# wlsdzyzl/OnePiece

Hardware: AMD Instinct MI355X
Metric: RGB-D frames/sec fused (640x480, 5 mm voxel TSDF) (higher is better)
Workload: dtype f32

## Files before the change

__graft_entry__.py:

```python
import os
import subprocess
import sys

ROOT = os.path.dirname(os.path.abspath(__file__))
if ROOT not in sys.path:
    sys.path.insert(0, ROOT)


def build():
    subprocess.check_call(["make", "-C", os.path.join(ROOT, "onepiece_amd", "csrc"), "-B", "-j8"])
    subprocess.check_call(["make", "-C", os.path.join(ROOT, "onepiece_amd", "csrc"), "-B", "-j8", "b64"])
    subprocess.check_call(["make", "-C", os.path.join(ROOT, "oracle"), "-B"])
    subprocess.check_call(["make", "-C", os.path.join(ROOT, "host", "one_piece"), "-B"])
    subprocess.check_call(["make", "-C", os.path.join(ROOT, "examples", "cpp"), "-B"])
    lib = os.path.join(ROOT, "onepiece_amd")
    subprocess.check_call(["/opt/rocm/bin/hipcc", "--offload-arch=gfx950", "-O2", "-I", os.path.join(ROOT, "include"), os.path.join(ROOT, "tools", "prof_driver.cpp"), "-L", lib,
                           "-lonepiece_hip", "-Wl,-rpath," + lib, "-o", os.path.join(ROOT, "tools", "prof_driver.bin")])
    hostlib = os.path.join(ROOT, "host", "one_piece")
    subprocess.check_call(["/opt/rocm/bin/hipcc", "--offload-arch=gfx950", "-O2", "-I", os.path.join(ROOT, "include"), os.path.join(ROOT, "tools", "ops_driver.cpp"), "-L", lib,
                           "-lonepiece_hip", "-L", hostlib, "-lone_piece_hip_host", "-Wl,-rpath," + lib, "-Wl,-rpath," + hostlib, "-o", os.path.join(ROOT, "tools", "ops_driver.bin")])
    for tool in ("hbm_calib", "valu_ubench"):
        subprocess.check_call(["/opt/rocm/bin/hipcc", "--offload-arch=gfx950", "-O2", "-Wno-unused-result", "-Wno-unused-value", os.path.join(ROOT, "tools", tool + ".hip"), "-o", os.path.join(ROOT, "tools", tool + ".bin")])
    try:
        subprocess.check_call(["make", "-C", os.path.join(ROOT, "tests", "cpp"), "-B"])
    except (OSError, subprocess.CalledProcessError) as e:
        print("build(): test artefacts under tests/cpp not built: %s" % e, file=sys.stderr)
    subprocess.check_call([os.path.join(ROOT, "oracle", "tools", "build_ref_examples.sh")])
    import onepiece_amd
    from onepiece_amd import _lib, integration, registration, odometry, dense_slam, distributed, sequence, synthetic, tool, nearest
    lib = _lib.load()
    assert lib.op_abi_version() == 1


def smoke():
    import numpy as np
    from onepiece_amd import integration as I, registration as R, synthetic as S
    from oracle import oracle as O

    s = 4
    camt = (S.FX / s, S.FY / s, S.CX / s, S.CY / s, S.W // s, S.H // s, 1000.0)
    hcam = I.PinholeCamera()
    hcam.fx, hcam.fy, hcam.cx, hcam.cy, hcam.width, hcam.height, hcam.depth_scale = camt
    hv = I.CubeHandler(hcam, device=0, max_blocks=1 << 15)
    hv.SetVoxelResolution(0.02)
# ... 46 lines not shown
```

include/onepiece_hip.h:

```cpp
#ifndef ONEPIECE_HIP_H
#define ONEPIECE_HIP_H
#include <stddef.h>
#include <stdint.h>

#ifdef __cplusplus
extern "C" {
#endif

#define OP_ABI_VERSION 1

typedef enum {
    OP_OK = 0,
    OP_ERR_INVALID = 1,
    OP_ERR_NO_DEVICE = 2,
    OP_ERR_CAPACITY = 3,
    OP_ERR_MISMATCH = 4,
    OP_ERR_NO_NORMALS = 5,
    OP_ERR_HIP = 6
} op_status;

enum { OP_DEPTH_F32 = 0, OP_DEPTH_U16 = 1 };
enum { OP_MEM_HOST = 0, OP_MEM_DEVICE = 1 };
enum { OP_ICP_POINT_TO_POINT = 0, OP_ICP_POINT_TO_PLANE = 1 };
enum { OP_TRACK_HYBRID = 0, OP_TRACK_PHOTO = 1, OP_TRACK_DEPTH = 2 };
// ... 33 lines not shown
#define OP_MERGE_OWNER_EXCHANGE 0
#define OP_MERGE_DENSE_REDUCE 1
int op_runtime_set_option(int option, long long value);
int op_runtime_get_option(int option, long long *value);
int op_runtime_set_rccl_library(const char *path);
int op_device_alloc(size_t bytes, int device, void **device_ptr);
int op_device_write(void *device_ptr, size_t n_parts, const void *const *parts, const size_t *bytes, const size_t *offsets, int device);
int op_device_upload(const void *host, size_t bytes, int device, void **device_ptr);
int op_device_release(void *device_ptr, int device);
int op_release_cached_memory(void);
int op_device_count(int *count);
int op_camera_preset(int type, op_camera *out);

int op_mat4_inverse(const float m[16], float out[16]);
uint64_t op_hash_key(int32_t x, int32_t y, int32_t z);
int op_frustum_planes(const op_camera *cam, const float pose[16], float far_dist, float near_dist,
                      float planes[24]);
int op_frustum_from_camera(const op_camera *cam, const float pose[16], float far_dist, float near_dist,
                           float planes[24], float corners[24]);
int op_frustum_from_vectors(const float forward[3], const float position[3], const float right[3],
                            const float up[3], float far_dist, float near_dist, float fov, float aspect,
                            float planes[24], float corners[24]);
int op_get_sdf(const op_camera *cam, const float point[3], const float pose[16], const float *pose_inv,
               const void *depth, int depth_fmt, float *sdf);
int op_debug_project_px(float a, float c, int fast);
int op_debug_project_uv(float fx, float fy, float cx, float cy, const float *X, const float *Y, const float *Z,
                        size_t n, int device, int32_t *out);
int op_debug_project_uv_image(float fx, float fy, float cx, float cy, int width, int height, const float *X, const float *Y,
                              const float *Z, size_t n, int device, int32_t *out);
int op_debug_voxel_update(const float *s, const float *w, const float *c0, const float *c1, const float *c2,
                          const float *new_sdf, const unsigned *rgba, long long n, float *out_fast, float *out_ref);
int op_debug_rcp(const float *x, long long n, float *out);
double op_debug_px_rcp_err(void);
int op_debug_gather2d(const unsigned *images, int width, int height, int n_frames, int frame, int column_test, const int *uv,
                      long long n, unsigned *out);
int op_se3_exp(const float x[6], float T[16]);

int op_volume_create(const op_camera *cam, float voxel_res, float truncation, float far_dist,
                     float near_dist, int device, uint64_t max_blocks, op_volume **out);
int op_volume_destroy(op_volume *v);
int op_volume_set_resolution(op_volume *v, float voxel_res);
int op_volume_set_truncation(op_volume *v, float truncation);
int op_volume_set_camera(op_volume *v, const op_camera *cam);
int op_volume_set_near_far(op_volume *v, float near_dist, float far_dist);
#define OP_VOLUME_OPT_UPDATE 0
#define OP_VOLUME_UPDATE_EXACT 0
#define OP_VOLUME_UPDATE_SUM_FORM 1
#define OP_VOLUME_OPT_SELECT 1
#define OP_VOLUME_SELECT_AUTO 0
#define OP_VOLUME_SELECT_DIRECT -1
#define OP_VOLUME_OPT_RAYCAST_PRUNE 2
int op_volume_set_option(op_volume *v, int option, int value);
int op_volume_progress(op_volume *v, uint64_t *frames_accepted, uint64_t *frames_done);
int op_volume_clear(op_volume *v);
int op_volume_sync(op_volume *v);
int op_volume_flush(op_volume *v);
int op_volume_block_count(op_volume *v, size_t *n);
int op_volume_has_cube(op_volume *v, int32_t x, int32_t y, int32_t z, int *present);
int op_volume_stream(op_volume *v, void **stream);

int op_volume_compute_bounding(op_volume *v, const void *depth, int depth_fmt, int mem,
                               const float pose[16], float max_pos[3], float min_pos[3],
                               size_t *n_inside);
int op_volume_prepare_cubes(op_volume *v, const void *depth, int depth_fmt, int mem,
                            const float pose[16], const float *pose_inv, int32_t *ids_xyz,
                            size_t cap, size_t *n, size_t *n_candidates);
// ... 248 lines not shown
```

onepiece_amd/_lib.py:

```python
import ctypes as C
import os
import subprocess

_HERE = os.path.dirname(os.path.abspath(__file__))
SO_PATH = os.environ.get("ONEPIECE_HIP_LIBRARY") or os.path.join(_HERE, "libonepiece_hip.so")
CSRC = os.path.join(_HERE, "csrc")


class OnePieceHipError(RuntimeError):
    def __init__(self, code, msg):
        super().__init__("onepiece_hip error %d: %s" % (code, msg))
        self.code = code


class Camera(C.Structure):
    _fields_ = [("fx", C.c_float), ("fy", C.c_float), ("cx", C.c_float), ("cy", C.c_float),
                ("width", C.c_int32), ("height", C.c_int32), ("depth_scale", C.c_float)]


class MergeStats(C.Structure):
    _fields_ = [("ranks", C.c_int32), ("rank", C.c_int32), ("union_blocks", C.c_uint64), ("reduce_bytes", C.c_uint64), ("slices", C.c_uint64),
                ("prepare_ms", C.c_double), ("transfer_ms", C.c_double), ("total_ms", C.c_double),
                ("algorithm", C.c_int32), ("pad_", C.c_int32), ("held_blocks", C.c_uint64), ("owned_blocks", C.c_uint64),
                ("wire_bytes_sent", C.c_uint64), ("wire_bytes_received", C.c_uint64)]
# ... 53 lines not shown
_ip = C.POINTER(C.c_int32)
_vp = C.c_void_p
_szp = C.POINTER(C.c_size_t)
_u64p = C.POINTER(C.c_uint64)

SIGNATURES = {
    "op_abi_version": (C.c_int, []),
    "op_last_error": (C.c_char_p, []),
    "op_runtime_hw_queues": (C.c_int, [C.POINTER(C.c_int)]),
    "op_runtime_configure": (C.c_int, [C.c_int]),
    "op_runtime_set_option": (C.c_int, [C.c_int, C.c_longlong]),
    "op_runtime_get_option": (C.c_int, [C.c_int, C.POINTER(C.c_longlong)]),
    "op_runtime_set_rccl_library": (C.c_int, [C.c_char_p]),
    "op_device_alloc": (C.c_int, [C.c_size_t, C.c_int, C.POINTER(_vp)]),
    "op_device_write": (C.c_int, [_vp, C.c_size_t, C.POINTER(_vp), C.POINTER(C.c_size_t), C.POINTER(C.c_size_t), C.c_int]),
    "op_device_upload": (C.c_int, [_vp, C.c_size_t, C.c_int, C.POINTER(_vp)]),
    "op_device_release": (C.c_int, [_vp, C.c_int]),
    "op_release_cached_memory": (C.c_int, []),
    "op_device_count": (C.c_int, [C.POINTER(C.c_int)]),
    "op_camera_preset": (C.c_int, [C.c_int, C.POINTER(Camera)]),
    "op_mat4_inverse": (C.c_int, [_fp, _fp]),
    "op_hash_key": (C.c_uint64, [C.c_int32, C.c_int32, C.c_int32]),
    "op_frustum_planes": (C.c_int, [C.POINTER(Camera), _fp, C.c_float, C.c_float, _fp]),
    "op_frustum_from_camera": (C.c_int, [C.POINTER(Camera), _fp, C.c_float, C.c_float, _fp, _fp]),
    "op_frustum_from_vectors": (C.c_int, [_fp, _fp, _fp, _fp, C.c_float, C.c_float, C.c_float, C.c_float, _fp, _fp]),
    "op_get_sdf": (C.c_int, [C.POINTER(Camera), _fp, _fp, _fp, _vp, C.c_int, _fp]),
    "op_se3_exp": (C.c_int, [_fp, _fp]),
    "op_debug_project_px": (C.c_int, [C.c_float, C.c_float, C.c_int]),
    "op_debug_project_uv": (C.c_int, [C.c_float, C.c_float, C.c_float, C.c_float, _vp, _vp, _vp, C.c_size_t, C.c_int, _vp]),
    "op_debug_project_uv_image": (C.c_int, [C.c_float, C.c_float, C.c_float, C.c_float, C.c_int, C.c_int, _vp, _vp, _vp, C.c_size_t, C.c_int, _vp]),
    "op_debug_voxel_update": (C.c_int, [_vp, _vp, _vp, _vp, _vp, _vp, _vp, C.c_longlong, _vp, _vp]),
    "op_debug_rcp": (C.c_int, [_vp, C.c_longlong, _vp]),
    "op_debug_px_rcp_err": (C.c_double, []),
    "op_debug_gather2d": (C.c_int, [_vp, C.c_int, C.c_int, C.c_int, C.c_int, C.c_int, _vp, C.c_longlong, _vp]),
    "op_volume_create": (C.c_int, [C.POINTER(Camera), C.c_float, C.c_float, C.c_float, C.c_float,
                                   C.c_int, C.c_uint64, C.POINTER(_vp)]),
    "op_volume_destroy": (C.c_int, [_vp]),
    "op_volume_set_resolution": (C.c_int, [_vp, C.c_float]),
    "op_volume_set_truncation": (C.c_int, [_vp, C.c_float]),
    "op_volume_set_camera": (C.c_int, [_vp, C.POINTER(Camera)]),
    "op_volume_set_near_far": (C.c_int, [_vp, C.c_float, C.c_float]),
    "op_volume_set_option": (C.c_int, [_vp, C.c_int, C.c_int]),
    "op_volume_progress": (C.c_int, [_vp, _u64p, _u64p]),
    "op_volume_clear": (C.c_int, [_vp]),
    "op_volume_sync": (C.c_int, [_vp]),
    "op_volume_flush": (C.c_int, [_vp]),
    "op_volume_block_count": (C.c_int, [_vp, _szp]),
    "op_volume_has_cube": (C.c_int, [_vp, C.c_int32, C.c_int32, C.c_int32, C.POINTER(C.c_int)]),
    "op_volume_stream": (C.c_int, [_vp, C.POINTER(_vp)]),
    "op_volume_compute_bounding": (C.c_int, [_vp, _vp, C.c_int, C.c_int, _fp, _fp, _fp, _szp]),
    "op_volume_prepare_cubes": (C.c_int, [_vp, _vp, C.c_int, C.c_int, _fp, _fp, _ip, C.c_size_t,
                                          _szp, _szp]),
    "op_volume_integrate": (C.c_int, [_vp, _vp, C.c_int, _vp, C.c_int, _fp, _fp]),
    "op_volume_integrate_sequence": (C.c_int, [_vp, _vp, C.c_size_t, C.c_int, _vp, C.c_size_t, _fp,
                                               C.c_size_t]),
    "op_volume_deintegrate": (C.c_int, [_vp, _vp, C.c_int, _vp, C.c_int, _fp, _fp]),
    "op_volume_deintegrate_sequence": (C.c_int, [_vp, _vp, C.c_size_t, C.c_int, _vp, C.c_size_t, _fp, C.c_size_t]),
    "op_volume_reintegrate": (C.c_int, [_vp, _vp, C.c_int, _vp, C.c_int, _fp, _fp]),
    "op_volume_reintegrate_sequence": (C.c_int, [_vp, _vp, C.c_size_t, C.c_int, _vp, C.c_size_t, _fp, _fp, C.c_size_t]),
    "op_volume_deintegrate_stats": (C.c_int, [_vp, _u64p, _u64p, _u64p, _u64p]),
    "op_volume_collect_garbage": (C.c_int, [_vp, C.c_float, _ip, _ip, C.POINTER(CollectStats)]),
    "op_volume_collect_last_stats": (C.c_int, [_vp, C.POINTER(CollectStats)]),
    "op_volume_integrate_cubes": (C.c_int, [_vp, _vp, C.c_int, _vp, C.c_int, _fp, _fp, _vp, C.c_size_t]),
    "op_volume_stats": (C.c_int, [_vp, _u64p, _u64p, _u64p, _u64p]),
    "op_volume_stats_launches": (C.c_int, [_vp, _u64p, _u64p, _u64p, _u64p]),
    "op_volume_growth_stats": (C.c_int, [_vp, _u64p, _u64p, _u64p]),
# ... 138 lines not shown
```

onepiece_amd/csrc/select.hip:

```cpp
#include "volume_core.hpp"

namespace {

__global__ void k_finish_select(VolView V, State* st) {
    for (unsigned k = blockIdx.x * blockDim.x + threadIdx.x; k < (unsigned)(kMaxBatch * kAccSlots * 8); k += gridDim.x * blockDim.x) (&st->acc[0][0][0])[k] = 0u;
    const unsigned n = st->n_blist < V.max_blocks ? st->n_blist : V.max_blocks;
    const unsigned nr = st->n_rec < V.max_blocks ? st->n_rec : V.max_blocks;
    for (unsigned i = blockIdx.x * blockDim.x + threadIdx.x; i < n; i += gridDim.x * blockDim.x) V.bmask[V.blist[i]] = (bmask_t)0;
    for (unsigned i = blockIdx.x * blockDim.x + threadIdx.x; i < nr; i += gridDim.x * blockDim.x) V.sel_list[i] = V.tvals[V.sel_list[i]];
}

__global__ void k_mark_cubes(VolView V, State* st, const int* __restrict__ keys, unsigned n) {
    const unsigned i = blockIdx.x * blockDim.x + threadIdx.x;
    if (i >= n || (st->overflow & 3u)) return;
    const int x = keys[3 * i], y = keys[3 * i + 1], z = keys[3 * i + 2];
    if (!key_in_range(x, y, z)) { atomicOr(&st->overflow, 8u); return; }
    bool created;
    const int slot = table_claim(V, st, x, y, z, &created);
    if (slot < 0) return;
    if (atomicOr(&V.bmask[slot], (bmask_t)1) == (bmask_t)0) {
        const unsigned pos = atomicAdd(&st->n_blist, 1u);
        if (pos < V.max_blocks) V.blist[pos] = slot;
    }
}



__global__ __launch_bounds__(256) void k_prepare_frames(KaFwd B, int f0, CamParams C, BatchPtrs Q, uint2* __restrict__ pimg, float2* __restrict__ ptile,
                                                        float* __restrict__ partial, State* st, unsigned seq,
                                                        const unsigned* __restrict__ n_blocks, unsigned* __restrict__ hstat) {
    __shared__ float s_red[4][6];
    __shared__ unsigned s_cnt[4];
    __shared__ float s_tile[4][4][2];
    const int tid = threadIdx.x, f = f0 + (int)blockIdx.y;
    if (blockIdx.x == 0 && f == 0 && tid == 0) {
        st->n_rec = 0;
        st->n_blist = 0;
        st->cur_seq = seq;
        if (hstat && (st->overflow & 3u) == 0u) {
            hstat[1] = *n_blocks;
            __threadfence_system();
            __hip_atomic_store(&hstat[0], seq - 1u, __ATOMIC_RELEASE, __HIP_MEMORY_SCOPE_SYSTEM);
        }
    }
    if (blockIdx.x == 0 && f == 0 && tid < kKcShares) st->kc_next[tid * 16] = 0u;
    if (blockIdx.x == 0 && f == 0) {
        static_assert(kKcTSlots == 256, "one slot per thread");
        unsigned long long kc = st->kc_t[tid];
        st->kc_t[tid] = 0ull;
        for (int o = 32; o > 0; o >>= 1) { const unsigned long long x = __shfl_xor(kc, o, 64); kc = x > kc ? x : kc; }
        __shared__ unsigned long long s_kc[4];
        if ((tid & 63) == 0) s_kc[tid >> 6] = kc;
        __syncthreads();
        if (tid == 0) {
            for (int w = 1; w < 4; ++w) kc = s_kc[w] > kc ? s_kc[w] : kc;
            st->stat_kc_ticks += kc;
        }
    }
    const PoseFwd& P = B.f[blockIdx.y];
    const int npix = C.width * C.height;
    const void* dptr = Q.depth[f];
    const unsigned char* cptr = Q.rgb[f];
    uint2* out = pimg + (size_t)f * npix;
    const int wgx = (C.width + kKaW - 1) / kKaW;
    const int gy = (int)blockIdx.x / wgx, gx = (int)blockIdx.x - gy * wgx;
    const int row = gy * kKaH + (tid >> 4), col0 = gx * kKaW + (tid & 15) * 4;
    float mx0 = -FLT_MAX, mx1 = -FLT_MAX, mx2 = -FLT_MAX, mn0 = FLT_MAX, mn1 = FLT_MAX, mn2 = FLT_MAX;
    float tmin = __builtin_inff(), tmax = -__builtin_inff();
    unsigned inside = 0;
    if (row < C.height && col0 < C.width) {
        const int pix0 = row * C.width + col0;
        float zz[4];
        unsigned cc[4] = {0u, 0u, 0u, 0u};
        const int nv = C.width - col0 < 4 ? C.width - col0 : 4;
        const bool wide = nv == 4 && (C.width & 3) == 0 && ((size_t)dptr & 15u) == 0 && ((size_t)cptr & 3u) == 0;
        if (wide) {
            if (C.depth_u16) {
                const ushort4 d = *reinterpret_cast<const ushort4*>((const unsigned short*)dptr + pix0);
                zz[0] = (float)d.x / C.depth_scale; zz[1] = (float)d.y / C.depth_scale; zz[2] = (float)d.z / C.depth_scale; zz[3] = (float)d.w / C.depth_scale;
            } else {
                const float4 d = *reinterpret_cast<const float4*>((const float*)dptr + pix0);
                zz[0] = d.x; zz[1] = d.y; zz[2] = d.z; zz[3] = d.w;
            }
            if (cptr) {
                const unsigned* c3 = reinterpret_cast<const unsigned*>(cptr + 3 * (size_t)pix0);
                const unsigned d0 = c3[0], d1 = c3[1], d2 = c3[2];
                cc[0] = d0 & 0xffffffu; cc[1] = (d0 >> 24) | ((d1 & 0xffffu) << 8); cc[2] = (d1 >> 16) | ((d2 & 0xffu) << 16); cc[3] = d2 >> 8;
            }
            uint4* o4 = reinterpret_cast<uint4*>(out + pix0);
            o4[0] = make_uint4(__float_as_uint(zz[0]), cc[0] | 0x01000000u, __float_as_uint(zz[1]), cc[1] | 0x01000000u);
            o4[1] = make_uint4(__float_as_uint(zz[2]), cc[2] | 0x01000000u, __float_as_uint(zz[3]), cc[3] | 0x01000000u);
        } else {
            for (int e = 0; e < nv; ++e) {
                const int pix = pix0 + e;
                zz[e] = C.depth_u16 ? (float)((const unsigned short*)dptr)[pix] / C.depth_scale : ((const float*)dptr)[pix];
                if (cptr) cc[e] = (unsigned)cptr[3 * (size_t)pix] | ((unsigned)cptr[3 * (size_t)pix + 1] << 8) | ((unsigned)cptr[3 * (size_t)pix + 2] << 16);
                out[pix] = make_uint2(__float_as_uint(zz[e]), cc[e] | 0x01000000u);
            }
        }
#pragma unroll
        for (int e = 0; e < 4; ++e) {
            if (e >= nv) break;
            const float z = zz[e];
            if (!(z > 0)) continue;
            tmin = fminf(tmin, z); tmax = fmaxf(tmax, z);
            const int i = row, j = col0 + e;
            const float x = ((float)j - C.cx) * z / C.fx;
            const float y = ((float)i - C.cy) * z / C.fy;
            const float* M = P.pose;
            const float q0 = ((M[0] * x + M[1] * y) + M[2] * z) + M[3] * 1.0f;
            const float q1 = ((M[4] * x + M[5] * y) + M[6] * z) + M[7] * 1.0f;
            const float q2 = ((M[8] * x + M[9] * y) + M[10] * z) + M[11] * 1.0f;
            const float q3 = ((M[12] * x + M[13] * y) + M[14] * z) + M[15] * 1.0f;
            float p0 = q0, p1 = q1, p2 = q2;
            if (__builtin_amdgcn_ballot_w64(q3 != 1.0f) != 0ull) { p0 = q0 / q3; p1 = q1 / q3; p2 = q2 / q3; }
            bool in = true;
#pragma unroll
            for (int k = 0; k < 6; ++k) {
                const float dist = sum3(P.planes[4 * k] * p0, P.planes[4 * k + 1] * p1, P.planes[4 * k + 2] * p2) + P.planes[4 * k + 3];
                if (dist < 0) { in = false; break; }
                if (dist == 0) break;
            }
            if (in) {
                ++inside;
                mx0 = p0 > mx0 ? p0 : mx0; mx1 = p1 > mx1 ? p1 : mx1; mx2 = p2 > mx2 ? p2 : mx2;
                mn0 = p0 < mn0 ? p0 : mn0; mn1 = p1 < mn1 ? p1 : mn1; mn2 = p2 < mn2 ? p2 : mn2;
            }
        }
    }
    tmin = fminf(tmin, __shfl_xor(tmin, 1, 64)); tmax = fmaxf(tmax, __shfl_xor(tmax, 1, 64));
    tmin = fminf(tmin, __shfl_xor(tmin, 2, 64)); tmax = fmaxf(tmax, __shfl_xor(tmax, 2, 64));
    tmin = fminf(tmin, __shfl_xor(tmin, 16, 64)); tmax = fmaxf(tmax, __shfl_xor(tmax, 16, 64));
    tmin = fminf(tmin, __shfl_xor(tmin, 32, 64)); tmax = fmaxf(tmax, __shfl_xor(tmax, 32, 64));
    mx0 = wave_max(mx0); mx1 = wave_max(mx1); mx2 = wave_max(mx2);
    mn0 = wave_min(mn0); mn1 = wave_min(mn1); mn2 = wave_min(mn2);
    inside = wave_sum(inside);
    const int wave = tid >> 6, lane = tid & 63;
    if (lane == 0) {
        s_red[wave][0] = mx0; s_red[wave][1] = mx1; s_red[wave][2] = mx2;
// ... 501 lines not shown
                    } else {
                        bool created;
                        const int ts = table_claim(V, st, bi, bj, bk, &created);
                        if (ts >= 0) {
                            if (!any_direct) { V.bmask[ts] = m; slot = ts; }
                            else if (atomicOr(&V.bmask[ts], m) == (bmask_t)0) slot = ts;
                        }
                    }
                }
            }
        }
        const unsigned long long got = __ballot(slot >= 0);
        if (lane == 0) s_wc[wave] = (unsigned)__popcll(got);
        if (__syncthreads_or(got != 0ull) == 0) continue;
        if (tid == 0) {
            unsigned n = 0;
            for (int w = 0; w < kMergeWords; ++w) { s_wp[w] = n; n += s_wc[w]; }
            s_base = atomicAdd(&st->n_blist, n);
        }
        __syncthreads();
        if (slot >= 0) {
            const unsigned pos = s_base + s_wp[wave] + (unsigned)__popcll(got & ((1ULL << lane) - 1ULL));
            if (pos < V.max_blocks) V.blist[pos] = slot;
        }
    }
}

}

namespace opv {

void launch_prepare_frames(op_volume* v, const BatchFwd& F, int nf, const CamParams& C, const BatchPtrs& Q, unsigned seq) {
    const int g1 = ka_grid(C.width, C.height);
    for (int f0 = 0; f0 < nf; f0 += kKaFrames) {
        KaFwd A;
        const int na = nf - f0 < kKaFrames ? nf - f0 : kKaFrames;
        std::memcpy(A.f, F.f + f0, sizeof(PoseFwd) * (size_t)na);
        hipLaunchKernelGGL(k_prepare_frames, dim3(g1, na), dim3(256), 0, v->stream, A, f0, C, Q, v->pimg, v->ptile, v->partial, v->state, seq,
                           (const unsigned*)v->n_blocks, v->hstat_dev);
    }
}

int launch_select(op_volume* v, const BatchInv& I, const CamParams& C, int nf, bool record, const int* cube_keys, unsigned n_cubes) {
    const VolView V = v->view();
    if (cube_keys)
        hipLaunchKernelGGL(k_mark_cubes, dim3((n_cubes + 255u) / 256u), dim3(256), 0, v->stream, V, v->state, cube_keys, n_cubes);
    else if (KB_VOTE && !record && nf >= (v->select_mode > 0 ? 2 : KB_VOTE_MIN_FRAMES) && v->select_mode != OP_VOLUME_SELECT_DIRECT) {
        if (!v->sbits) OP_HIP(op::cached_malloc((void**)&v->sbits, (size_t)kMaxBatch * kVoteCap * sizeof(unsigned long long)));
        const unsigned vote_cap = v->select_mode > 0 ? (unsigned)v->select_mode : kVoteCap;
        const int per_frame = std::max(8, std::min(kSelectGrid, (KB_VOTE_WGS / nf + 7) / 8 * 8));
        if (C.fast_px)
            hipLaunchKernelGGL(k_select_vote<true>, dim3(per_frame, nf), dim3(256), 0, v->stream, I, C, V, (const uint2*)v->pimg, (const float2*)v->ptile, v->state, v->sbits, vote_cap);
        else
            hipLaunchKernelGGL(k_select_vote<false>, dim3(per_frame, nf), dim3(256), 0, v->stream, I, C, V, (const uint2*)v->pimg, (const float2*)v->ptile, v->state, v->sbits, vote_cap);
        hipLaunchKernelGGL(k_select_merge, dim3(KB_MERGE_GRID), dim3(64 * kMergeWords), 0, v->stream, V, v->state, (const unsigned long long*)v->sbits, nf);
    } else if (C.fast_px)
        hipLaunchKernelGGL(k_select<true>, dim3(kSelectGrid, nf), dim3(256), 0, v->stream, I, C, V, (const uint2*)v->pimg, (const float2*)v->ptile,
                           v->state, record ? 1 : 0);
    else
        hipLaunchKernelGGL(k_select<false>, dim3(kSelectGrid, nf), dim3(256), 0, v->stream, I, C, V, (const uint2*)v->pimg, (const float2*)v->ptile,
                           v->state, record ? 1 : 0);
    return OP_OK;
}

void launch_finish_select(op_volume* v) { hipLaunchKernelGGL(k_finish_select, dim3(256), dim3(256), 0, v->stream, v->view(), v->state); }

void kb_trace_dump(op_volume* v) {
#ifdef KB_TRACE
    if (hipSetDevice(v->device) == hipSuccess && hipDeviceSynchronize() == hipSuccess) {
        const int nw = std::max(8, std::min(kSelectGrid, (KB_VOTE_WGS / kMaxBatch + 7) / 8 * 8)) * kMaxBatch * 4;
        std::vector<unsigned long long> t((size_t)nw * 8);
        if (hipMemcpyFromSymbol(t.data(), HIP_SYMBOL(g_kb_trace), t.size() * 8) == hipSuccess) {
            double sum[8] = {0}, mx[8] = {0}, tot_max = 0, tot_sum = 0;
            std::vector<double> tots;
            for (int w = 0; w < nw; ++w) {
                double tot = 0;
                for (int k = 0; k < 8; ++k) { const double d = (double)t[(size_t)w * 8 + k]; sum[k] += d; mx[k] = std::max(mx[k], d); if (k < 4) tot += d; }
                tot_max = std::max(tot_max, tot); tot_sum += tot; tots.push_back(tot);
            }
            std::sort(tots.begin(), tots.end());
            const double n = nw;
            fprintf(stderr, "kb trace (shader cycles, %d waves; mean/max): total %.0f/%.0f (median %.0f, 90%% %.0f, 99%% %.0f) setup %.0f/%.0f coarse %.0f/%.0f exact %.0f/%.0f barrier %.0f/%.0f | rounds %.2f/%.0f exact tests %.2f/%.0f\n",
                    nw, tot_sum / n, tot_max, tots[tots.size() / 2], tots[tots.size() * 9 / 10], tots[tots.size() * 99 / 100], sum[0] / n, mx[0], sum[1] / n, mx[1], sum[2] / n, mx[2], sum[3] / n, mx[3], sum[4] / n, mx[4], sum[5] / n, mx[5]);
        }
    }
#else
    (void)v;
#endif
}

}
```

onepiece_amd/csrc/volume.hip:

```cpp
#include "volume_core.hpp"

namespace op {
thread_local char g_last_error[512] = "";
}

namespace op {
RuntimeOptions& runtime_options() { static RuntimeOptions o; return o; }
}

namespace {

__global__ void k_debug_project_uv(CamParams C, const float* __restrict__ X, const float* __restrict__ Y,
                                   const float* __restrict__ Z, size_t n, int* __restrict__ out) {
    const size_t i = blockIdx.x * (size_t)blockDim.x + threadIdx.x;
    if (i >= n) return;
    const int pix = C.fast_px ? project_pixel<true>(C, X[i], Y[i], Z[i]) : project_pixel<false>(C, X[i], Y[i], Z[i]);
    out[4 * i] = pix < 0 ? INT_MIN : pix % C.width;
    out[4 * i + 1] = pix < 0 ? INT_MIN : pix / C.width;
    out[4 * i + 2] = px_round_dp((C.fx * X[i]) / Z[i], C.cx);
    out[4 * i + 3] = px_round_dp((C.fy * Y[i]) / Z[i], C.cy);
}

__global__ void k_fill_pool(float* pool, size_t first_block, size_t n_blocks) {
    const size_t total = n_blocks * kBlockFloats;
// ... 643 lines not shown

int op_device_count(int* count) {
    if (!count) return fail(OP_ERR_INVALID, "null count");
    int n = 0;
    hipError_t e = hipGetDeviceCount(&n);
    *count = e == hipSuccess ? n : 0;
    return OP_OK;
}

int op_camera_preset(int type, op_camera* out) {
    if (!out) return fail(OP_ERR_INVALID, "null camera");
    if (type == 0) *out = op_camera{517.3f, 516.5f, 318.6f, 255.3f, 640, 480, 5000.0f};
    else if (type == 1) *out = op_camera{514.817f, 515.375f, 318.771f, 238.447f, 640, 480, 1000.0f};
    else return fail(OP_ERR_INVALID, "unknown camera preset %d", type);
    return OP_OK;
}

int op_mat4_inverse(const float m[16], float out[16]) {
    if (!m || !out) return fail(OP_ERR_INVALID, "null matrix");
    op_host::mat4_inverse(m, out);
    return OP_OK;
}

uint64_t op_hash_key(int32_t x, int32_t y, int32_t z) { return op_host::hash_key(x, y, z); }

int op_frustum_planes(const op_camera* cam, const float pose[16], float far_dist, float near_dist, float planes[24]) {
    OP_TRY(check_cam(cam));
    if (!pose || !planes) return fail(OP_ERR_INVALID, "null argument");
    op_host::CameraPOD c{cam->fx, cam->fy, cam->cx, cam->cy, cam->width, cam->height, cam->depth_scale};
    op_host::frustum_planes(c, pose, far_dist, near_dist, planes);
    return OP_OK;
}

int op_frustum_from_camera(const op_camera* cam, const float pose[16], float far_dist, float near_dist, float planes[24], float corners[24]) {
    OP_TRY(check_cam(cam));
    if (!pose || !planes) return fail(OP_ERR_INVALID, "null argument");
    op_host::CameraPOD c{cam->fx, cam->fy, cam->cx, cam->cy, cam->width, cam->height, cam->depth_scale};
    op_host::frustum_planes(c, pose, far_dist, near_dist, planes, corners);
    return OP_OK;
}

int op_frustum_from_vectors(const float forward[3], const float position[3], const float right[3], const float up[3], float far_dist, float near_dist,
                            float fov, float aspect, float planes[24], float corners[24]) {
    if (!forward || !position || !right || !up || !planes) return fail(OP_ERR_INVALID, "null argument");
    op_host::frustum_from_vectors(forward, position, right, up, far_dist, near_dist, fov, aspect, planes, corners);
    return OP_OK;
}

int op_get_sdf(const op_camera* cam, const float point[3], const float pose[16], const float* pose_inv, const void* depth, int depth_fmt, float* sdf) {
    OP_TRY(check_cam(cam));
    if (!point || !pose || !depth || !sdf) return fail(OP_ERR_INVALID, "null argument");
    float inv[16];
    if (pose_inv) std::memcpy(inv, pose_inv, sizeof(inv));
    else op_host::mat4_inverse(pose, inv);
    float q[3];
    for (int r = 0; r < 3; ++r) q[r] = ((inv[4 * r] * point[0] + inv[4 * r + 1] * point[1]) + inv[4 * r + 2] * point[2]) + inv[4 * r + 3] * 1.0f;
    const int u = px_round_dp((cam->fx * q[0]) / q[2], cam->cx);
    const int w = px_round_dp((cam->fy * q[1]) / q[2], cam->cy);
    *sdf = 999.0f;
    if (w < 0 || w >= cam->height || u < 0 || u >= cam->width) return OP_OK;
    const size_t at = (size_t)w * cam->width + u;
    const float d = depth_fmt == OP_DEPTH_U16 ? (float)((const unsigned short*)depth)[at] / cam->depth_scale : ((const float*)depth)[at];
    if (d <= 0) return OP_OK;
    *sdf = d - q[2];
    return OP_OK;
}
// ... 544 lines not shown
```

onepiece_amd/csrc/volume_core.hpp:

```cpp
#pragma once
#include <cfloat>
#include <climits>
#include <algorithm>
#include <numeric>
#include <vector>

#include <atomic>
#include <condition_variable>
#include <deque>
#include <memory>
#include <mutex>
#include <thread>

#include "common.hpp"

#include <type_traits>
#include "host_math.hpp"
#include "px_round.hpp"

namespace opv {

using op::fail;

constexpr int kVox = 512;
constexpr int kBlockFloats = 5 * kVox;
constexpr unsigned long long kEmptyKey = ~0ULL;
constexpr int kPending = -1;
constexpr int kDead = -3;
constexpr int kKaW = 64, kKaH = 16;
constexpr int kTile = 16;
#ifndef KB_GRID
#define KB_GRID 384
#endif
constexpr int kSelectGrid = KB_GRID;
static_assert(kSelectGrid % 8 == 0 && kSelectGrid >= 8, "k_select deals a frame's workgroups to the 8 XCDs in equal shares");
#ifndef OP_MAX_BATCH
#define OP_MAX_BATCH 32
#endif
constexpr int kMaxBatch = OP_MAX_BATCH;
constexpr int kKaFrames = 16;
static_assert(kMaxBatch <= 64 && kMaxBatch % kKaFrames == 0, "one bit of the batch mask per frame; KA takes kKaFrames frames per launch");
typedef std::conditional<(kMaxBatch > 32), unsigned long long, unsigned>::type bmask_t;
__host__ __device__ inline int mask_ctz(unsigned m) { return __builtin_ctz(m); }
__host__ __device__ inline int mask_ctz(unsigned long long m) { return __builtin_ctzll(m); }
__device__ inline unsigned mask_popc(unsigned m) { return (unsigned)__popc(m); }
__device__ inline unsigned mask_popc(unsigned long long m) { return (unsigned)__popcll(m); }
constexpr int kAccSlots = 16;
#ifndef KC_ZT
#define KC_ZT 2
#endif
#ifndef KC_COL_MIN_WAVES
// ... 1 lines not shown
#endif
#ifndef KC_COL_GRID
#define KC_COL_GRID (256 * KC_COL_MIN_WAVES * 4 / (8 / KC_ZT))
#endif
constexpr int kColGrid = KC_COL_GRID;
#ifndef KC_ZT_SUM
#define KC_ZT_SUM 2
#endif
#ifndef KC_SUM_MIN_WAVES
#define KC_SUM_MIN_WAVES KC_COL_MIN_WAVES
#endif
constexpr int kColGridSum = 256 * KC_SUM_MIN_WAVES * 4 / (8 / KC_ZT_SUM);
static_assert(kColGridSum % 8 == 0, "one drawing workgroup per XCD slab at least");
static_assert(kColGrid % 8 == 0, "one drawing workgroup per XCD slab at least");
#ifndef KC_SIGNED_MIN_WAVES
#define KC_SIGNED_MIN_WAVES 7
#endif
constexpr int kSignedGrid = 256 * KC_SIGNED_MIN_WAVES * 4 / (8 / KC_ZT);
static_assert(kSignedGrid % 8 == 0, "one drawing workgroup per XCD slab at least");
constexpr int kPartialGrid = 1024;
constexpr int kDeiReverted = 0, kDeiReset = kPartialGrid, kDeiSkipped = 2 * kPartialGrid, kDeiFrames = 3 * kPartialGrid;
constexpr int kCoordLimit = 1 << 20;

struct CamParams {
    float fx, fy, cx, cy, depth_scale, res, trunc;
    int width, height, depth_u16;
    PxAxis ax, ay;
    int fast_px;
};
struct PoseFwd { float pose[16]; float planes[24]; };
struct PoseInv { float m[12]; };
struct BatchFwd { PoseFwd f[kMaxBatch]; };
struct KaFwd { PoseFwd f[kKaFrames]; };
struct BatchInv { PoseInv f[kMaxBatch]; };
struct BatchPtrs { const void* depth[kMaxBatch]; const unsigned char* rgb[kMaxBatch]; };

constexpr int kKcShares = 8;
#ifndef KC_STEAL_MIN_FRAMES
#define KC_STEAL_MIN_FRAMES 24
#endif
constexpr int kKcTSlots = 256;
struct State {
    unsigned pad0;
    unsigned overflow;
    unsigned n_rec;
    unsigned fail_seq;
    unsigned cur_seq;
    unsigned pad[3];
    unsigned long long stat_frames;
    unsigned long long stat_launches;
    unsigned long long kc_t[kKcTSlots];
    unsigned long long stat_kc_ticks;
    unsigned long long n_cand[kMaxBatch];
    float bbox[kMaxBatch][6];
    unsigned n_inside[kMaxBatch];
    unsigned acc[kMaxBatch][kAccSlots][8];
    unsigned kc_next[kKcShares * 16];
    unsigned n_blist;
    unsigned pad1[7];
    int sel_rng[kMaxBatch][8];
};

struct StateHead { unsigned pad0, overflow, n_rec, fail_seq, cur_seq, pad[3]; };
static_assert(sizeof(StateHead) == 32 && offsetof(State, stat_frames) == 32, "StateHead mirrors the head of State");

struct VolView {
// ... 356 lines not shown
```

Measured before the change: 59040.

## Replace per-pixel divisions with certified reciprocal-multiply fast path in frame prep

Adds a host-side certificate that proves, per frame, a pixel rectangle and depth window where a reciprocal multiply plus one FMA correction gives bit-identical results to IEEE division, and that points there lie inside the frustum planes. k_prepare_frames gets a templated fast path that uses this cheaper division for depth scaling and back-projection and skips the frustum plane tests inside the certified region. The aim is to cut the costly f32 divisions and plane checks in the prepare kernel. In exchange it adds host work per launch (certificate computation, memoized quotient checks), larger kernel arguments, and more complex correctness reasoning; a trace build variant is also added.

```diff
diff --git a/__graft_entry__.py b/__graft_entry__.py
--- a/__graft_entry__.py
+++ b/__graft_entry__.py
@@ -10,6 +10,7 @@
 def build():
     subprocess.check_call(["make", "-C", os.path.join(ROOT, "onepiece_amd", "csrc"), "-B", "-j8"])
     subprocess.check_call(["make", "-C", os.path.join(ROOT, "onepiece_amd", "csrc"), "-B", "-j8", "b64"])
+    subprocess.check_call(["make", "-C", os.path.join(ROOT, "onepiece_amd", "csrc"), "-j8", "katrace"])
     subprocess.check_call(["make", "-C", os.path.join(ROOT, "oracle"), "-B"])
     subprocess.check_call(["make", "-C", os.path.join(ROOT, "host", "one_piece"), "-B"])
     subprocess.check_call(["make", "-C", os.path.join(ROOT, "examples", "cpp"), "-B"])
diff --git a/include/onepiece_hip.h b/include/onepiece_hip.h
--- a/include/onepiece_hip.h
+++ b/include/onepiece_hip.h
@@ -89,6 +89,7 @@
                           const float *new_sdf, const unsigned *rgba, long long n, float *out_fast, float *out_ref);
 int op_debug_rcp(const float *x, long long n, float *out);
 double op_debug_px_rcp_err(void);
+int op_debug_ka_certificate(const op_camera *cam, const float pose[16], float far_dist, float near_dist, int32_t rect[4], float z[2], int32_t quot[3]);
 int op_debug_gather2d(const unsigned *images, int width, int height, int n_frames, int frame, int column_test, const int *uv,
                       long long n, unsigned *out);
 int op_se3_exp(const float x[6], float T[16]);
diff --git a/onepiece_amd/_lib.py b/onepiece_amd/_lib.py
--- a/onepiece_amd/_lib.py
+++ b/onepiece_amd/_lib.py
@@ -109,6 +109,7 @@
     "op_debug_voxel_update": (C.c_int, [_vp, _vp, _vp, _vp, _vp, _vp, _vp, C.c_longlong, _vp, _vp]),
     "op_debug_rcp": (C.c_int, [_vp, C.c_longlong, _vp]),
     "op_debug_px_rcp_err": (C.c_double, []),
+    "op_debug_ka_certificate": (C.c_int, [C.POINTER(Camera), _fp, C.c_float, C.c_float, _vp, _fp, _vp]),
     "op_debug_gather2d": (C.c_int, [_vp, C.c_int, C.c_int, C.c_int, C.c_int, C.c_int, _vp, C.c_longlong, _vp]),
     "op_volume_create": (C.c_int, [C.POINTER(Camera), C.c_float, C.c_float, C.c_float, C.c_float,
                                    C.c_int, C.c_uint64, C.POINTER(_vp)]),
diff --git a/onepiece_amd/csrc/ka_cert.hpp b/onepiece_amd/csrc/ka_cert.hpp
--- /dev/null
+++ b/onepiece_amd/csrc/ka_cert.hpp
@@ -0,0 +1,183 @@
+#pragma once
+#include <algorithm>
+#include <cfloat>
+#include <cmath>
+#include <cstdint>
+#include <cstring>
+
+#include "px_round.hpp"
+
+struct KaQuot {
+    float y;
+    int ok;
+    int lo, hi;
+};
+struct KaCert { int j_lo, j_hi, i_lo, i_hi; float z_lo, z_hi; };
+struct KaCam { KaQuot qx, qy, qd; };
+
+constexpr double kKaOrthoTol = 1.0e-4;
+
+OP_HD float ka_div_const(float n, float b, float y) {
+    const float q0 = n * y;
+    const float r = __builtin_fmaf(-b, q0, n);
+    return __builtin_fmaf(r, y, q0);
+}
+
+namespace ka_detail {
+inline uint32_t bits_of(float f) { uint32_t u; std::memcpy(&u, &f, 4); return u; }
+inline int exponent_of(float f) { return (int)((bits_of(f) >> 23) & 0xffu) - 127; }
+inline uint32_t inv_odd(uint32_t a) { uint32_t x = a; for (int k = 0; k < 5; ++k) x *= 2u - a * x; return x; }
+constexpr int kKaMaxD = 8;
+template <class F>
+inline void risky_numerators(uint32_t B, F&& f) {
+    const int tz = __builtin_ctz(B);
+    if (tz > 3) return;
+    const uint32_t Bo = B >> tz;
+    for (int kind = 0; kind < 2; ++kind) {
+        const int sh = kind == 0 ? 25 : 24;
+        const uint64_t m2 = (1ull << sh) >> tz;
+        for (int D = -kKaMaxD; D <= kKaMaxD; ++D) {
+            if (D == 0 || (D & ((1 << tz) - 1)) != 0) continue;
+            const int64_t rhs = -(int64_t)(D / (1 << tz));
+            const uint64_t K0 = ((uint64_t)(uint32_t)((uint32_t)rhs * inv_odd(Bo))) & (m2 - 1);
+            for (uint64_t K = K0; K < (1ull << 25); K += m2) {
+                if (K < (1ull << 24) || (K & 1ull) == 0) continue;
+                const int64_t num = (int64_t)((uint64_t)B * K) + D;
+                if ((num & (int64_t)((1ull << sh) - 1)) != 0) continue;
+                const int64_t N = num >> sh;
+                if (N >= (1 << 23) && N < (1 << 24)) f((uint32_t)N);
+            }
+        }
+    }
+}
+}
+
+inline KaQuot ka_quot(float b) {
+    using namespace ka_detail;
+    KaQuot q{0.0f, 0, 0, -1};
+    if (!(b > 0.0f) || !std::isfinite(b) || (bits_of(b) >> 23) == 0u) return q;
+    const float y = 1.0f / b;
+    q.y = y;
+    if (!std::isfinite(y) || (bits_of(y) >> 23) == 0u) return q;
+    const double by = std::fma((double)b, (double)y, -1.0);
+    const double bl = std::fma((double)b, (double)std::nextafterf(y, 0.0f), -1.0), bh = std::fma((double)b, (double)std::nextafterf(y, INFINITY), -1.0);
+    if (!(std::fabs(by) < std::fabs(bl) && std::fabs(by) < std::fabs(bh))) return q;
+    const uint32_t frac = bits_of(b) & 0x7fffffu;
+    if (frac == 0x7fffffu) return q;
+    const int eb = exponent_of(b);
+    const uint32_t B = frac | 0x800000u;
+    const int tz = __builtin_ctz(B);
+    const float bs = std::ldexp(1.0f, eb - 23);
+    bool same = true;
+    risky_numerators(B, [&](uint32_t N) {
+        const float n = (float)N * bs;
+        same = same && bits_of(ka_div_const(n, b, y)) == bits_of(n / b) && bits_of(ka_div_const(-n, b, y)) == bits_of(-n / b);
+    });
+    if (!same) return q;
+    q.lo = eb - 125 > -79 - tz ? eb - 125 : -79 - tz;
+    q.hi = eb >= 0 ? 127 : 127 + eb;
+    q.ok = q.lo <= q.hi;
+    return q;
+}
+
+inline KaCam ka_cam(float fx, float fy, float depth_scale) { return KaCam{ka_quot(fx), ka_quot(fy), ka_quot(depth_scale)}; }
+
+inline bool ka_axis_in_window(float c, int lo, int hi, float z_lo, float z_hi, const KaQuot& Q) {
+    double amin = INFINITY, amax = 0.0;
+    const double fl = std::floor((double)c);
+    const double cand[5] = {(double)lo, (double)hi, fl - 1.0, fl, fl + 1.0};
+    for (double j : cand) {
+        if (j < lo || j > hi) continue;
+        const float a = (float)j - c;
+        const double m = std::fabs((double)a);
+        if (m != 0.0 && m < amin) amin = m;
+        if (m > amax) amax = m;
+    }
+    if (amax == 0.0) return true;
+    return amin * (double)z_lo >= std::ldexp(1.0, Q.lo + 1) && amax * (double)z_hi < std::ldexp(1.0, Q.hi);
+}
+
+inline KaCert ka_certificate(const float pose[16], const float planes[24], float fx, float fy, float cx, float cy, int width, int height, const KaCam& Q,
+                             double e_scale = 1.0, bool whole_image = false) {
+    const KaCert none{0, -1, 0, -1, 1.0f, 0.0f};
+    if (!Q.qx.ok || !Q.qy.ok || width <= 0 || height <= 0) return none;
+    if (!(pose[12] == 0.0f && pose[13] == 0.0f && pose[14] == 0.0f && pose[15] == 1.0f)) return none;
+    double mag = 0.0;
+    for (int k = 0; k < 12; ++k) mag += std::fabs((double)pose[k]);
+    for (int k = 0; k < 24; ++k) mag += std::fabs((double)planes[k]);
+    if (!std::isfinite(mag) || !(fx > 0.0f) || !(fy > 0.0f) || !std::isfinite(cx) || !std::isfinite(cy)) return none;
+    double M[3][4];
+    for (int r = 0; r < 3; ++r)
+        for (int c = 0; c < 4; ++c) M[r][c] = (double)pose[4 * r + c];
+    for (int a = 0; a < 3; ++a)
+        for (int b = a; b < 3; ++b) {
+            const double s = M[0][a] * M[0][b] + M[1][a] * M[1][b] + M[2][a] * M[2][b] - (a == b ? 1.0 : 0.0);
+            if (!(std::fabs(s) <= kKaOrthoTol)) return none;
+        }
+    const double u = 0x1p-24;
+    const double g1 = u / (1 - u), g4 = 4 * u / (1 - 4 * u), g7 = 7 * u / (1 - 7 * u);
+    const double A = std::fmax(std::fabs(0.0 - (double)cx), std::fabs((double)(width - 1) - (double)cx)) / (double)fx;
+    const double Bm = std::fmax(std::fabs(0.0 - (double)cy), std::fabs((double)(height - 1) - (double)cy)) / (double)fy;
+    double c0[6], c1[6], c2[6], dc[6], E0[6], E1[6];
+    for (int k = 0; k < 6; ++k) {
+        const double n[3] = {(double)planes[4 * k], (double)planes[4 * k + 1], (double)planes[4 * k + 2]}, d = (double)planes[4 * k + 3];
+        if (std::fabs(n[0]) > 2.0 || std::fabs(n[1]) > 2.0 || std::fabs(n[2]) > 2.0) return none;
+        double nc[3], sS = 0.0, sT = 0.0;
+        for (int c = 0; c < 3; ++c) nc[c] = M[0][c] * n[0] + M[1][c] * n[1] + M[2][c] * n[2];
+        for (int r = 0; r < 3; ++r) {
+            sS += std::fabs(n[r]) * (std::fabs(M[r][0]) * A + std::fabs(M[r][1]) * Bm + std::fabs(M[r][2]));
+            sT += std::fabs(n[r]) * std::fabs(M[r][3]);
+        }
+        c0[k] = nc[0] / (double)fx; c1[k] = nc[1] / (double)fy; c2[k] = nc[2];
+        dc[k] = (n[0] * M[0][3] + n[1] * M[1][3] + n[2] * M[2][3]) + d;
+        E1[k] = e_scale * ((g4 + (1 + g4) * g7) * sS + 0x1p-44 * sS);
+        E0[k] = e_scale * ((g4 + (1 + g4) * g1) * sT + g1 * std::fabs(d) + 0x1p-44 * (sT + std::fabs(d)) + 0x1p-120);
+    }
+    const auto g = [&](int k, double j, double i) { return c0[k] * (j - (double)cx) + c1[k] * (i - (double)cy) + c2[k]; };
+    const auto gmin = [&](int k, int jl, int jh, int il, int ih) {
+        return std::fmin(std::fmin(g(k, jl, il), g(k, jh, il)), std::fmin(g(k, jl, ih), g(k, jh, ih)));
+    };
+    double zl = 0x1p-60, zh = 0x1p60;
+    for (int k = 4; k < 6; ++k) {
+        const double s = gmin(k, 0, width - 1, 0, height - 1) - E1[k], off = dc[k] - E0[k];
+        if (s > 0) { if (off < 0) zl = std::fmax(zl, -off / s); }
+        else if (s < 0) { if (!(off > 0)) return none; zh = std::fmin(zh, off / -s); }
+        else if (!(off > 0)) return none;
+    }
+    float z_lo = (float)zl, z_hi = (float)zh;
+    if ((double)z_lo < zl) z_lo = std::nextafterf(z_lo, INFINITY);
+    if ((double)z_hi > zh) z_hi = std::nextafterf(z_hi, 0.0f);
+    z_lo = std::nextafterf(z_lo, INFINITY); z_hi = std::nextafterf(z_hi, 0.0f);
+    if (!(z_lo > 0.0f) || !(z_lo <= z_hi)) return none;
+    if (whole_image) return KaCert{0, width - 1, 0, height - 1, z_lo, z_hi};
+    int jl = 0, jh = width - 1, il = 0, ih = height - 1;
+    for (int k = 0; k < 4; ++k) {
+        const double need = E1[k] + std::fmax((E0[k] - dc[k]) / (double)z_lo, 0.0) + 0x1p-40;
+        if (std::fabs(c0[k]) * width >= std::fabs(c1[k]) * height) {
+            if (c0[k] == 0.0) return none;
+            const double w = std::fmin(c1[k] * (0.0 - (double)cy), c1[k] * ((double)(height - 1) - (double)cy));
+            const double lim = (double)cx + (need - c2[k] - w) / c0[k];
+            if (!std::isfinite(lim) || std::fabs(lim) > 1.0e9) return none;
+            if (c0[k] > 0) jl = std::max(jl, (int)std::ceil(lim)); else jh = std::min(jh, (int)std::floor(lim));
+        } else {
+            const double w = std::fmin(c0[k] * (0.0 - (double)cx), c0[k] * ((double)(width - 1) - (double)cx));
+            const double lim = (double)cy + (need - c2[k] - w) / c1[k];
+            if (!std::isfinite(lim) || std::fabs(lim) > 1.0e9) return none;
+            if (c1[k] > 0) il = std::max(il, (int)std::ceil(lim)); else ih = std::min(ih, (int)std::floor(lim));
+        }
+    }
+    for (int attempt = 0; attempt < 2; ++attempt) {
+        if (jl > jh || il > ih) return none;
+        bool ok = true;
+        for (int k = 0; k < 6 && ok; ++k) {
+            const double s = gmin(k, jl, jh, il, ih) - E1[k], off = dc[k] - E0[k];
+            ok = s * (double)z_lo + off > 0 && s * (double)z_hi + off > 0;
+        }
+        if (ok) {
+            if (!ka_axis_in_window(cx, jl, jh, z_lo, z_hi, Q.qx) || !ka_axis_in_window(cy, il, ih, z_lo, z_hi, Q.qy)) return none;
+            return KaCert{jl, jh, il, ih, z_lo, z_hi};
+        }
+        ++jl; --jh; ++il; --ih;
+    }
+    return none;
+}
diff --git a/onepiece_amd/csrc/select.hip b/onepiece_amd/csrc/select.hip
--- a/onepiece_amd/csrc/select.hip
+++ b/onepiece_amd/csrc/select.hip
@@ -26,9 +26,20 @@
 
 
 
+#ifdef KA_TRACE
+__device__ unsigned long long g_ka_waves[2];
+#define KA_COUNT(K) do { if (__lane_id() == (unsigned)__builtin_ctzll(__builtin_amdgcn_read_exec())) atomicAdd(&g_ka_waves[K], 1ull); } while (0)
+#else
+#define KA_COUNT(K) do { } while (0)
+#endif
+
+struct KaNoArgs {};
+template <bool KAFAST>
 __global__ __launch_bounds__(256) void k_prepare_frames(KaFwd B, int f0, CamParams C, BatchPtrs Q, uint2* __restrict__ pimg, float2* __restrict__ ptile,
                                                         float* __restrict__ partial, State* st, unsigned seq,
-                                                        const unsigned* __restrict__ n_blocks, unsigned* __restrict__ hstat) {
+                                                        const unsigned* __restrict__ n_blocks, unsigned* __restrict__ hstat,
+                                                        typename std::conditional<KAFAST, KaArgs, KaNoArgs>::type KA) {
+    const KaArgs* const K = KAFAST ? reinterpret_cast<const KaArgs*>(&KA) : nullptr;
     __shared__ float s_red[4][6];
     __shared__ unsigned s_cnt[4];
     __shared__ float s_tile[4][4][2];
@@ -77,7 +88,12 @@
         if (wide) {
             if (C.depth_u16) {
                 const ushort4 d = *reinterpret_cast<const ushort4*>((const unsigned short*)dptr + pix0);
-                zz[0] = (float)d.x / C.depth_scale; zz[1] = (float)d.y / C.depth_scale; zz[2] = (float)d.z / C.depth_scale; zz[3] = (float)d.w / C.depth_scale;
+                if (KAFAST && K->use_d) {
+                    zz[0] = ka_div_const((float)d.x, C.depth_scale, K->yd); zz[1] = ka_div_const((float)d.y, C.depth_scale, K->yd);
+                    zz[2] = ka_div_const((float)d.z, C.depth_scale, K->yd); zz[3] = ka_div_const((float)d.w, C.depth_scale, K->yd);
+                } else {
+                    zz[0] = (float)d.x / C.depth_scale; zz[1] = (float)d.y / C.depth_scale; zz[2] = (float)d.z / C.depth_scale; zz[3] = (float)d.w / C.depth_scale;
+                }
             } else {
                 const float4 d = *reinterpret_cast<const float4*>((const float*)dptr + pix0);
                 zz[0] = d.x; zz[1] = d.y; zz[2] = d.z; zz[3] = d.w;
@@ -93,10 +109,20 @@
         } else {
             for (int e = 0; e < nv; ++e) {
                 const int pix = pix0 + e;
-                zz[e] = C.depth_u16 ? (float)((const unsigned short*)dptr)[pix] / C.depth_scale : ((const float*)dptr)[pix];
+                if (KAFAST && C.depth_u16 && K->use_d) zz[e] = ka_div_const((float)((const unsigned short*)dptr)[pix], C.depth_scale, K->yd);
+                else zz[e] = C.depth_u16 ? (float)((const unsigned short*)dptr)[pix] / C.depth_scale : ((const float*)dptr)[pix];
                 if (cptr) cc[e] = (unsigned)cptr[3 * (size_t)pix] | ((unsigned)cptr[3 * (size_t)pix + 1] << 8) | ((unsigned)cptr[3 * (size_t)pix + 2] << 16);
                 out[pix] = make_uint2(__float_as_uint(zz[e]), cc[e] | 0x01000000u);
             }
+        }
+        bool crow = false;
+        int cj = 0, cw = -1;
+        float cz_lo = 0.0f, cz_hi = 0.0f;
+        if (KAFAST) {
+            const KaCert& T = K->c[blockIdx.y];
+            crow = row >= T.i_lo && row <= T.i_hi;
+            cj = col0 - T.j_lo; cw = T.j_hi - T.j_lo;
+            cz_lo = T.z_lo; cz_hi = T.z_hi;
         }
 #pragma unroll
         for (int e = 0; e < 4; ++e) {
@@ -105,6 +131,22 @@
             if (!(z > 0)) continue;
             tmin = fminf(tmin, z); tmax = fmaxf(tmax, z);
             const int i = row, j = col0 + e;
+            if (KAFAST) {
+                KA_COUNT(0);
+                if (crow & ((unsigned)(cj + e) <= (unsigned)cw) & (z >= cz_lo) & (z <= cz_hi)) {
+                    const float x = ka_div_const(((float)j - C.cx) * z, C.fx, K->yx);
+                    const float y = ka_div_const(((float)i - C.cy) * z, C.fy, K->yy);
+                    const float* M = P.pose;
+                    const float p0 = ((M[0] * x + M[1] * y) + M[2] * z) + M[3] * 1.0f;
+                    const float p1 = ((M[4] * x + M[5] * y) + M[6] * z) + M[7] * 1.0f;
+                    const float p2 = ((M[8] * x + M[9] * y) + M[10] * z) + M[11] * 1.0f;
+                    ++inside;
+                    mx0 = p0 > mx0 ? p0 : mx0; mx1 = p1 > mx1 ? p1 : mx1; mx2 = p2 > mx2 ? p2 : mx2;
+                    mn0 = p0 < mn0 ? p0 : mn0; mn1 = p1 < mn1 ? p1 : mn1; mn2 = p2 < mn2 ? p2 : mn2;
+                    continue;
+                }
+                KA_COUNT(1);
+            }
             const float x = ((float)j - C.cx) * z / C.fx;
             const float y = ((float)i - C.cy) * z / C.fy;
             const float* M = P.pose;
@@ -672,12 +714,32 @@
 
 void launch_prepare_frames(op_volume* v, const BatchFwd& F, int nf, const CamParams& C, const BatchPtrs& Q, unsigned seq) {
     const int g1 = ka_grid(C.width, C.height);
+    static thread_local struct { float fx, fy, ds; KaCam cam; bool set; } memo;
+    if (!memo.set || memo.fx != C.fx || memo.fy != C.fy || memo.ds != C.depth_scale) {
+        memo.fx = C.fx; memo.fy = C.fy; memo.ds = C.depth_scale; memo.cam = ka_cam(C.fx, C.fy, C.depth_scale); memo.set = true;
+    }
+    const KaCam& QC = memo.cam;
     for (int f0 = 0; f0 < nf; f0 += kKaFrames) {
         KaFwd A;
         const int na = nf - f0 < kKaFrames ? nf - f0 : kKaFrames;
         std::memcpy(A.f, F.f + f0, sizeof(PoseFwd) * (size_t)na);
-        hipLaunchKernelGGL(k_prepare_frames, dim3(g1, na), dim3(256), 0, v->stream, A, f0, C, Q, v->pimg, v->ptile, v->partial, v->state, seq,
-                           (const unsigned*)v->n_blocks, v->hstat_dev);
+        KaArgs K;
+        bool any = false;
+        for (int k = 0; k < kKaFrames; ++k) {
+            K.c[k] = k < na ? ka_certificate(A.f[k].pose, A.f[k].planes, C.fx, C.fy, C.cx, C.cy, C.width, C.height, QC) : KaCert{0, -1, 0, -1, 1.0f, 0.0f};
+            any = any || K.c[k].j_lo <= K.c[k].j_hi;
+        }
+#ifdef KA_TRACE
+        any = true;
+#endif
+        K.yx = QC.qx.y; K.yy = QC.qy.y; K.yd = QC.qd.y;
+        K.use_d = C.depth_u16 && QC.qd.ok && QC.qd.lo <= 0 && QC.qd.hi >= 15;
+        if (any)
+            hipLaunchKernelGGL(k_prepare_frames<true>, dim3(g1, na), dim3(256), 0, v->stream, A, f0, C, Q, v->pimg, v->ptile, v->partial, v->state, seq,
+                               (const unsigned*)v->n_blocks, v->hstat_dev, K);
+        else
+            hipLaunchKernelGGL(k_prepare_frames<false>, dim3(g1, na), dim3(256), 0, v->stream, A, f0, C, Q, v->pimg, v->ptile, v->partial, v->state, seq,
+                               (const unsigned*)v->n_blocks, v->hstat_dev, KaNoArgs{});
     }
 }
 
@@ -727,6 +789,21 @@
 #else
     (void)v;
 #endif
-}
-
-}
+#ifdef KA_TRACE
+    unsigned long long w[2] = {0, 0};
+    if (hipSetDevice(v->device) == hipSuccess && hipDeviceSynchronize() == hipSuccess && hipMemcpyFromSymbol(w, HIP_SYMBOL(g_ka_waves), sizeof(w)) == hipSuccess)
+        fprintf(stderr, "KA_TRACE k_prepare_frames<true>: %llu wave passes over a pixel slot with a valid lane, %llu of them through the full sequence (%.3f %%)\n", w[0], w[1],
+                w[0] ? 100.0 * (double)w[1] / (double)w[0] : 0.0);
+#endif
+}
+
+}
+
+#ifdef KA_TRACE
+extern "C" __attribute__((visibility("default"))) int op_debug_ka_trace(unsigned long long out[2], int reset) {
+    if (hipDeviceSynchronize() != hipSuccess || hipMemcpyFromSymbol(out, HIP_SYMBOL(g_ka_waves), 16) != hipSuccess) return -1;
+    const unsigned long long zero[2] = {0, 0};
+    if (reset && hipMemcpyToSymbol(HIP_SYMBOL(g_ka_waves), zero, 16) != hipSuccess) return -1;
+    return 0;
+}
+#endif
diff --git a/onepiece_amd/csrc/volume.hip b/onepiece_amd/csrc/volume.hip
--- a/onepiece_amd/csrc/volume.hip
+++ b/onepiece_amd/csrc/volume.hip
@@ -699,6 +699,20 @@
     return OP_OK;
 }
 
+int op_debug_ka_certificate(const op_camera* cam, const float pose[16], float far_dist, float near_dist, int32_t rect[4], float z[2], int32_t quot[3]) {
+    OP_TRY(check_cam(cam));
+    if (!pose || !rect || !z || !quot) return fail(OP_ERR_INVALID, "null argument");
+    op_host::CameraPOD c{cam->fx, cam->fy, cam->cx, cam->cy, cam->width, cam->height, cam->depth_scale};
+    float planes[24];
+    op_host::frustum_planes(c, pose, far_dist, near_dist, planes);
+    const KaCam Q = ka_cam(cam->fx, cam->fy, cam->depth_scale);
+    const KaCert T = ka_certificate(pose, planes, cam->fx, cam->fy, cam->cx, cam->cy, cam->width, cam->height, Q);
+    rect[0] = T.j_lo; rect[1] = T.j_hi; rect[2] = T.i_lo; rect[3] = T.i_hi;
+    z[0] = T.z_lo; z[1] = T.z_hi;
+    quot[0] = Q.qx.ok; quot[1] = Q.qy.ok; quot[2] = Q.qd.ok && Q.qd.lo <= 0 && Q.qd.hi >= 15;
+    return OP_OK;
+}
+
 int op_frustum_from_camera(const op_camera* cam, const float pose[16], float far_dist, float near_dist, float planes[24], float corners[24]) {
     OP_TRY(check_cam(cam));
     if (!pose || !planes) return fail(OP_ERR_INVALID, "null argument");
diff --git a/onepiece_amd/csrc/volume_core.hpp b/onepiece_amd/csrc/volume_core.hpp
--- a/onepiece_amd/csrc/volume_core.hpp
+++ b/onepiece_amd/csrc/volume_core.hpp
@@ -17,6 +17,7 @@
 #include <type_traits>
 #include "host_math.hpp"
 #include "px_round.hpp"
+#include "ka_cert.hpp"
 
 namespace opv {
 
@@ -84,6 +85,8 @@
 struct PoseInv { float m[12]; };
 struct BatchFwd { PoseFwd f[kMaxBatch]; };
 struct KaFwd { PoseFwd f[kKaFrames]; };
+struct KaArgs { KaCert c[kKaFrames]; float yx, yy, yd; int use_d; };
+static_assert(sizeof(KaArgs) == 24 * kKaFrames + 16, "six words per frame");
 struct BatchInv { PoseInv f[kMaxBatch]; };
 struct BatchPtrs { const void* depth[kMaxBatch]; const unsigned char* rgb[kMaxBatch]; };
 
```

After: 59850 (median of 6 runs). 1.01x the previous value.
